# HasnainRaz/Fast-SRGAN

Hardware: AMD Instinct MI355X
Metric: SR train-step images/sec (96->384 4x, full GAN step: G+D+VGG perceptual loss) (higher is better)
Workload: dtype x3v; 1 GPU; BASELINE configs[2]: full GAN training step, 8 residual blocks / 64 filters, 96x96->384x384; per_gpu_batch=32, global_batch=32, parallelism=dp1, collectives=none, rccl_world_size=1, launch=hipGraph replay

## Files before the change

### fast-srgan_amd/_lib.py

```python
import ctypes
import os

_HERE = os.path.dirname(os.path.abspath(__file__))
LIB_PATH = os.environ.get("FSR_HIP_LIB") or os.path.join(_HERE, "libfsr_hip.so")

FSR_F32, FSR_BF16, FSR_F16, FSR_X3 = 0, 1, 2, 3
ACT_NONE, ACT_RELU, ACT_LEAKY, ACT_PRELU, ACT_TANH = 0, 1, 2, 3, 4
CONV_FWD, CONV_DGRAD = 0, 1
PACK_FWD, PACK_FWD_PS, PACK_DGRAD, PACK_DGRAD_PS = 0, 1, 2, 3
OUT_DTYPE, OUT_F32, OUT_U8, OUT_I420 = 0, 1, 2, 3
YUV_BT601, YUV_BT709 = 0, 1
SITING_JPEG, SITING_MPEG2 = 0, 1
OPT_BIAS, OPT_PRELU, OPT_OSCALE, OPT_MASK, OPT_PREACT, OPT_STATS = 1, 2, 4, 8, 16, 32
ABI_VERSION = 11

c_int, c_float, c_void_p, c_size_t, c_ll = ctypes.c_int, ctypes.c_float, ctypes.c_void_p, ctypes.c_size_t, ctypes.c_longlong


class ConvDesc(ctypes.Structure):
    _fields_ = [
        ("dtype", c_int), ("mode", c_int),
        ("n", c_int), ("ih", c_int), ("iw", c_int), ("cin", c_int),
        ("oh", c_int), ("ow", c_int), ("cout", c_int),
        ("stride", c_int), ("act", c_int), ("slope", c_float),
        ("pixel_shuffle", c_int), ("in_pixel_shuffled", c_int), ("out_f32", c_int), ("pool2", c_int), ("mask_is_addend", c_int), ("pack_lin", c_int),
        ("yuv_matrix", c_int), ("yuv_full_range", c_int),
    ]


# ... 9 lines not shown
P = c_void_p
SIGNATURES = {
    "fsr_version": (c_int, []),
    "fsr_last_error": (ctypes.c_char_p, []),
    "fsr_last_kernel": (ctypes.c_char_p, []),
    "fsr_device_info": (c_int, [ctypes.c_char_p, c_size_t]),
    "fsr_pack_conv3x3": (c_int, [c_int, c_int, P, c_int, c_int, c_int, P, P]),
    "fsr_pack_conv3x3_lin": (c_int, [c_int, c_int, P, c_int, c_int, c_int, P, P]),
    "fsr_conv3x3_pack_block": (c_int, [ctypes.POINTER(ConvDesc), c_int]),
    "fsr_conv3x3_scratch": (c_size_t, [ctypes.POINTER(ConvDesc)]),
    "fsr_conv3x3": (c_int, [ctypes.POINTER(ConvDesc), P, P, P, P, P, P, c_float, P, P, P, P, P]),
    "fsr_conv3x3_wgrad_workspace": (c_size_t, [ctypes.POINTER(WgradDesc)]),
    "fsr_conv3x3_wgrad": (c_int, [ctypes.POINTER(WgradDesc), P, P, P, P, P]),
    "fsr_conv3x3_wgrad_grouped_workspace": (c_size_t, [ctypes.POINTER(WgradDesc), c_int]),
    "fsr_conv3x3_wgrad_grouped": (c_int, [ctypes.POINTER(WgradDesc), c_int, P, P, P, P, P]),
    "fsr_instnorm_act_fwd": (c_int, [c_int, P, P, P, c_int, c_float, P, P, c_int, c_int, c_int, P]),
    "fsr_instnorm_act_bwd_scratch": (c_size_t, [c_int, c_int, c_int]),
    "fsr_instnorm_act_bwd_reduce": (c_int, [c_int, P, P, P, c_int, c_float, P, P, P, P, c_int, c_int, c_int, P]),
    "fsr_instnorm_act_bwd_apply": (c_int, [c_int, P, P, P, P, c_int, c_float, P, P, c_int, c_int, c_int, P]),
    "fsr_act_bwd_scratch": (c_size_t, [c_int, c_int, c_int, c_int, c_int]),
    "fsr_act_bwd": (c_int, [c_int, P, P, c_int, c_float, P, P, P, P, P, c_int, c_int, c_int, c_int, c_int, P]),
    "fsr_add": (c_int, [c_int, P, P, P, c_ll, P]),
    "fsr_image_to_nhwc": (c_int, [c_int, P, c_ll, c_ll, c_ll, c_ll, c_int, c_int, c_int, c_float, c_float, c_float,
                                  c_float, c_float, c_float, P, c_int, P]),
    "fsr_u8_to_image": (c_int, [P, P, c_ll, P]),
    "fsr_i420_to_image": (c_int, [P, P, c_int, c_int, c_int, c_int, c_int, c_int, P]),
    "fsr_pack_conv3x3_c3": (c_int, [c_int, P, c_int, P, c_int, P]),
    "fsr_tanh_bwd_image": (c_int, [P, c_ll, c_ll, c_ll, c_ll, P, c_int, c_int, c_int, P, P, P, P]),
    "fsr_conv3x3_c3_fwd": (c_int, [c_int, P, c_ll, c_ll, c_ll, c_ll, c_int, c_int, c_int, c_float, c_float, c_float, c_float,
                                   c_float, c_float, P, P, c_int, c_float, P, c_int, P, P, P, P]),
# ... 72 lines not shown
```

### fast-srgan_amd/csrc/conv_c3.hip

```cpp
#include "fsr_common.h"
#include "fsr_host.h"

namespace {

struct C3Args {
  const float* img;
  long long sn, sc, sh, sw;
  int N, H, W;
  float scale[3], shift[3];
  const void* wpk;
  const float* bias;
  const float* prelu;
  int act;
  float slope;
  int cout;
  void* out;
  void* preact;
  unsigned char* signs;
  const void* dz;
  float* ws;
  int tiles_x, tiles_y, tiles_per_slab, ntiles;
};

constexpr int PW = 18;
// ... 154 lines not shown
        for (int t = 0; t < 4; ++t) {
          acc[t] = (f32x4){0.f, 0.f, 0.f, 0.f};
#pragma unroll
          for (int j = 0; j < 8; ++j) acc[t] = mfma_f32_16x16x4(wf32[t][j], xv[j], acc[t]);
        }
        if (gx < a.W && gy < a.H) {
          const size_t off = (((size_t)n * a.H + gy) * a.W + gx) * a.cout + nb * 64 + lg * 8;
#pragma unroll
          for (int p = 0; p < 2; ++p) {
            const f32x4 lo = acc[2 * p] + bv[2 * p], hi = acc[2 * p + 1] + bv[2 * p + 1];
            float v8[8] = {lo[0], lo[1], lo[2], lo[3], hi[0], hi[1], hi[2], hi[3]};
            if (prep) V16<x3_t, 4>::st((x3_t*)prep + off + p * 32, v8);
#pragma unroll
            for (int q = 0; q < 8; ++q) v8[q] = fmaxf(v8[q], 0.f) + slope * fminf(v8[q], 0.f);
            V16<x3_t, 4>::st((x3_t*)outp + off + p * 32, v8);
          }
        }
        continue;
      }
    }
    static_for<0, 4>([&](auto tc) {
      constexpr int t = decltype(tc)::value;
      if (t < ntile) {
        f32x4 acc = (f32x4){0.f, 0.f, 0.f, 0.f};
        if constexpr (sizeof(T) == 2) {
          acc = mfma16<T>(wf16[t], xf16, acc);
        } else {
#pragma unroll
          for (int j = 0; j < 8; ++j) acc = mfma_f32_16x16x4(wf32[t][j], xv[j], acc);
        }
// ... 228 lines not shown
                                  void* preact, void* signs, fsr_stream_t stream_) {
  C3Args a = {};
  const float scale3[3] = {scale0, scale1, scale2}, shift3[3] = {shift0, shift1, shift2};
  if (int rc = fill_args(a, "fsr_conv3x3_c3_fwd", dtype, img, sn, sc, sh, sw, n, h, w, scale3, shift3, cout)) return rc;
  if (!packed_w || !out) return fsr_fail(-1, "fsr_conv3x3_c3_fwd: null argument");
  if (act == FSR_ACT_PRELU && !prelu_weight) return fsr_fail(-1, "fsr_conv3x3_c3_fwd: PReLU needs its weight");
  if (act == FSR_ACT_TANH) return fsr_fail(-2, "fsr_conv3x3_c3_fwd: tanh is not a first-layer activation");
  a.wpk = packed_w;
  a.bias = bias;
  a.prelu = prelu_weight;
  a.act = act;
  a.slope = slope;
  a.out = out;
  a.preact = preact;
  if (dtype == FSR_X3 && ((((size_t)out | (size_t)preact) & 127) != 0)) return fsr_fail(-2, "fsr_conv3x3_c3_fwd: x3 tensors must be 128-byte aligned");
  if (signs && (dtype == FSR_F32 || dtype == FSR_X3 || cout % 64 != 0)) return fsr_fail(-2, "fsr_conv3x3_c3_fwd: sign bits are written by the 16-bit kernels for cout %% 64 == 0");
  a.signs = (unsigned char*)signs;
  a.tiles_x = (w + 15) / 16;
  a.tiles_y = (h + 15) / 16;
  const long long nwg = (long long)a.tiles_x * a.tiles_y * n;
  if (nwg > 0x7fffffffLL) return fsr_fail(-2, "fsr_conv3x3_c3_fwd: bad grid");
  const dim3 grid((unsigned)nwg, (unsigned)((cout + 63) / 64));
  if (dtype == FSR_BF16) hipLaunchKernelGGL(conv_c3_fwd_kernel<bf16_t>, grid, dim3(256), 0, (hipStream_t)stream_, a);
  else if (dtype == FSR_F16) hipLaunchKernelGGL(conv_c3_fwd_kernel<f16_t>, grid, dim3(256), 0, (hipStream_t)stream_, a);
  else if (dtype == FSR_X3) hipLaunchKernelGGL((conv_c3_fwd_kernel<float, x3_t>), grid, dim3(256), 0, (hipStream_t)stream_, a);
  else hipLaunchKernelGGL(conv_c3_fwd_kernel<float>, grid, dim3(256), 0, (hipStream_t)stream_, a);
  return fsr_check_launch("conv_c3_fwd_kernel");
}

static int c3_wgrad_slabs(int n, int h, int w, int* tiles_x, int* tiles_y, int* per) {
  *tiles_x = (w + 15) / 16;
// ... 38 lines not shown
```

### fast-srgan_amd/csrc/conv_s2d3.hip

```cpp
#include "fsr_common.h"
#include "fsr_conv_args.h"
#include "fsr_host.h"

#include <stdlib.h>

#ifndef FSR_ABLS
#define FSR_ABLS 0
#endif

namespace {

constexpr int S2D_ABL = FSR_ABLS;

typedef float f32x16 __attribute__((ext_vector_type(16)));

template <typename T> struct Mfma32;
template <> struct Mfma32<bf16_t> {
  static __device__ __forceinline__ f32x16 run(s16x8 a, s16x8 b, f32x16 c) {
    return __builtin_amdgcn_mfma_f32_32x32x16_bf16(__builtin_bit_cast(bf16x8_hw, a), __builtin_bit_cast(bf16x8_hw, b), c, 0, 0, 0);
  }
};
template <> struct Mfma32<f16_t> {
  static __device__ __forceinline__ f32x16 run(s16x8 a, s16x8 b, f32x16 c) {
    return __builtin_amdgcn_mfma_f32_32x32x16_f16(__builtin_bit_cast(f16x8_hw, a), __builtin_bit_cast(f16x8_hw, b), c, 0, 0, 0);
// ... 381 lines not shown
    attr_set = true;
  }
  long long grid = (long long)s2d_cus() * 2;
  if (grid > a.t3_ntiles) grid = a.t3_ntiles;
  hipLaunchKernelGGL(kern, dim3((unsigned)grid), dim3(S2D_NW * 64), S2D_LDS, stream, a);
  fsr_note_kernel("conv_s2d3_kernel<%s>", X3 ? "x3" : (std::is_same<T, f16_t>::value ? "f16" : "bf16"));
  const int rc = fsr_check_launch("conv_s2d3_kernel");
  return rc ? rc : 1;
}

}

int fsr_conv_s2d3_try(int dtype, ConvKArgs& a, hipStream_t stream) {
  static const bool off = getenv("FSR_S2D3") && atoi(getenv("FSR_S2D3")) == 0;
  if (off || (dtype != FSR_BF16 && dtype != FSR_F16 && dtype != FSR_X3)) return 0;
  if (dtype == FSR_X3 && ((a.Cin & 63) != 0 || (a.Cin >> 6) * 3 >= (1 << 15) || a.dmask_bits)) return 0;
  if (a.Cin < 64 || a.Cin % 32 != 0 || a.Cout % 64 != 0 || a.Cout < 64 || a.CoutPad != a.Cout) return 0;
  if (a.ps || a.in_ps || a.out_f32 || a.preact || a.oscale || a.bias || a.stats || a.pool2 || a.act != FSR_ACT_NONE || a.dmask_add) return 0;
  if (a.IH != (a.FOH - 1) / 2 + 1 || a.IW != (a.FOW - 1) / 2 + 1) return 0;
  if ((long long)a.N * a.IH * a.IW * a.Cin >= (1LL << 31) || (long long)a.N * a.FOH * a.FOW * a.Cout >= (1LL << 31)) return 0;
  ConvKArgs b = a;
  b.tiles_x = (b.IW + 15) / 16;
  b.tiles_y = (b.IH + S2D_TH - 1) / S2D_TH;
  b.nblk_n = b.Cout / S2D_BN;
  const long long ntiles = (long long)b.tiles_x * b.tiles_y * b.N * b.nblk_n;
  if (ntiles <= 0 || ntiles > 0x7fffffffLL) return 0;
  b.t3_ntiles = (int)ntiles;
  const int want = b.Cin >= 128 ? S2D_BN : 0;
  if (b.query) {
    a.wlin_want = want;
    return 1;
// ... 9 lines not shown
```

### fast-srgan_amd/csrc/conv_tall3_body.h

```cpp
#pragma once
#include "fsr_common.h"
#include "fsr_conv_args.h"
#include "fsr_host.h"

#include <stdlib.h>

#ifndef FSR_ABL3
#define FSR_ABL3 0
#endif


int fsr_t3_cus();

namespace {

constexpr int T3_ABL = FSR_ABL3;

typedef float f32x16 __attribute__((ext_vector_type(16)));

template <typename T> struct Mfma32;
template <> struct Mfma32<bf16_t> {
  static __device__ __forceinline__ f32x16 run(s16x8 a, s16x8 b, f32x16 c) {
    return __builtin_amdgcn_mfma_f32_32x32x16_bf16(__builtin_bit_cast(bf16x8_hw, a), __builtin_bit_cast(bf16x8_hw, b), c, 0, 0, 0);
  }
// ... 402 lines not shown
        if constexpr (ACT == FSR_ACT_RELU) return fmaxf(x, 0.f);
        else if constexpr (ACT == FSR_ACT_LEAKY) return fmaxf(x, x * slope);
        else if constexpr (ACT == FSR_ACT_PRELU) return x > 0.f ? x : x * slope;
        else return x;
      };
      static_for<0, NA>([&](auto nc) {
        constexpr int n = decltype(nc)::value;
        const int co = onb * BN + wco * (NA * 32) + n * 32 + hi * 16;
        static_for<0, MB>([&](auto mc) {
          constexpr int m = decltype(mc)::value;
          const int gy = ogy0 + wpx * 2 * MB + 2 * m + lrow;
          const bool ok = gy < a.GH && gx < a.GW;
          float v[16];
#pragma unroll
          for (int e = 0; e < 16; ++e) v[e] = acc[n][m][e];
          if (a.pool2) {
#pragma unroll
            for (int e = 0; e < 16; ++e) {
              float x = v[e];
              x = fmaxf(x, __shfl_xor(x, 16, 64));
              x = fmaxf(x, __shfl_xor(x, 1, 64));
              v[e] = activate(x);
            }
            if (!(T3_ABL & 1) && ok && lrow == 0 && !(l15 & 1)) {
              const unsigned off = (unsigned)((oimg * (a.FOH >> 1) + (gy >> 1)) * (a.FOW >> 1) + (gx >> 1)) * (unsigned)a.Cout + (unsigned)co;
              store16(outp + off, v, [](float x) { return x; });
            }
          } else if (!(T3_ABL & 1) && ok) {
            unsigned off = (unsigned)((oimg * a.FOH + gy) * a.FOW + gx) * (unsigned)a.Cout + (unsigned)co;
            if constexpr (UP) {
              if (ps_out) {
                const int q = co >> a.t3_ps_shift, cc = co - (q << a.t3_ps_shift);
                off = (unsigned)((oimg * 2 * a.FOH + 2 * gy + (q >> 1)) * (2 * a.FOW) + 2 * gx + (q & 1)) * (unsigned)(a.Cout >> 2) + (unsigned)cc;
              }
              if (prep) store16(prep + off, v, [](float x) { return x; });
            }

            if (maskp) {
              const char* mp = X3 ? (const char*)x3_hi_ptr(maskp + off) : (const char*)(maskp + off);
              const u32x4 k0 = *(const u32x4*)mp, k1 = *(const u32x4*)(mp + 16);
              const float ms = a.dmask_slope;
              if (a.dmask_add) {
                if constexpr (X3) {
                  const u32x4 q0 = *(const u32x4*)(mp + 64), q1 = *(const u32x4*)(mp + 80);
#pragma unroll
                  for (int e = 0; e < 4; ++e) {
                    v[2 * e] += x3_join_lo(k0[e], q0[e]);
                    v[2 * e + 1] += x3_join_hi(k0[e], q0[e]);
                    v[8 + 2 * e] += x3_join_lo(k1[e], q1[e]);
                    v[8 + 2 * e + 1] += x3_join_hi(k1[e], q1[e]);
                  }
                } else {
#pragma unroll
// ... 134 lines not shown
```

### fast-srgan_amd/csrc/conv_wgrad.hip

```cpp
#include "fsr_common.h"
#include "fsr_host.h"
#include <cstdlib>

constexpr int WGRAD_GROUP_MAX = 32;

#ifndef FSR_ABLW
#define FSR_ABLW 0
#endif

struct WgradKArgs {
  const void* x;
  const void* dy;
  float* ws;
  int N, IH, IW, CinPad;
  int OH, OW, CoutPad;
  int dy_ps;
  int tiles_x, tiles_y, tiles_total, tiles_per_slab, nslab;
  int nbm, nbn;
  int x3;
  int group_n;
  const void* gx[WGRAD_GROUP_MAX];
  const void* gdy[WGRAD_GROUP_MAX];
};

// ... 29 lines not shown
  constexpr int PA = BM + PAD, PB = BN + PAD;
  constexpr int HH = (TPH - 1) * S + 3, HW = 15 * S + 3;
  constexpr int NPAIR = (BM / 16) * (BN / 16);
  constexpr int TPW = (NPAIR + NW - 1) / NW;
  constexpr int NBT = BN / 16;
  static_assert(TPW <= NBT, "a wave's pairs must share its co tile");
  constexpr int TPIX = TPH * 16;

  HIP_DYNAMIC_SHARED(char, smem)
  T* dyt = (T*)smem;
  T* halo = dyt + TPIX * PA;
  constexpr bool DMA = wgrad_dma<T, BM, BN, S, TPH>();

  const int tid = threadIdx.x, lane = tid & 63, wave = __builtin_amdgcn_readfirstlane(tid >> 6);
  const int l15 = lane & 15, lg = lane >> 4;
  int bid = a.group_n > 0 ? (int)blockIdx.x : xcd_remap((int)blockIdx.x, (int)gridDim.x);
  const int layer = a.group_n > 0 ? bid / a.nslab : 0;
  if (a.group_n > 0) bid -= layer * a.nslab;
  const int bn = bid % a.nbn;
  bid /= a.nbn;
  const int bm = bid % a.nbm;
  const int slab = bid / a.nbm;

  constexpr bool COPAIR = (BM >= 64 && BN == 64);
  const bool active = wave * TPW < NPAIR;
  const int co_t = COPAIR ? (wave / NBT) * TPW : (wave * TPW) / NBT;
  constexpr bool x3blk = X3W;
  const int ci_t0 = COPAIR ? (x3blk ? (wave + 2 * (wave / NBT)) % NBT : wave % NBT) : (wave * TPW) % NBT;
  const bool skip_lo = x3blk && ci_t0 >= 2;

  f32x4 acc[9][TPW];
#pragma unroll
  for (int t = 0; t < 9; ++t)
// ... 286 lines not shown
            acc[t][1] = mfma_f32_16x16x4(av1, bv, acc[t][1]);
          } else {
#pragma unroll
            for (int j = 0; j < TPW; ++j) acc[t][j] = mfma_f32_16x16x4(av, pb[j * 16], acc[t][j]);
          }
        }
      }
    }
  }

  if (!active) return;
#pragma unroll
  for (int t = 0; t < 9; ++t)
#pragma unroll
    for (int j = 0; j < TPW; ++j) {
      const int cot = COPAIR ? co_t + j : co_t, cit = COPAIR ? ci_t0 : ci_t0 + j;
      float* o = a.ws + (((size_t)(layer * a.nslab + slab) * 9 + t) * a.CoutPad + bm * BM + cot * 16 + lg * 4) * a.CinPad + bn * BN + cit * 16 + l15;
#pragma unroll
      for (int r = 0; r < 4; ++r) o[(size_t)r * a.CinPad] = acc[t][j][r];
    }
}

__global__ __launch_bounds__(256) void conv_wgrad_reduce_kernel(const float* __restrict__ ws, float* __restrict__ dw, int nslab,
                                                                int cout, int cin, int cout_pad, int cin_pad, int ps) {
  __shared__ float red[8][32];
  const int total = 9 * cout * cin;
  const size_t sstride = (size_t)9 * cout_pad * cin_pad;
  const int oi = threadIdx.x & 31, pl = threadIdx.x >> 5;
  for (int i0 = blockIdx.x * 32; i0 < total; i0 += gridDim.x * 32) {
    const int i = i0 + oi;
// ... 209 lines not shown
      const float* p = wl + ((size_t)t * cout_pad + co) * cin_pad + ci;
      for (int k = pl; k < nslab; k += 8) s += p[(size_t)k * sstride];
    }
    red[pl][oi] = s;
    __syncthreads();
    if (pl == 0 && i < total) {
      float r = red[0][oi];
#pragma unroll
      for (int j = 1; j < 8; ++j) r += red[j][oi];
      dw[((size_t)co * cin + ci) * 9 + t] += r;
    }
    __syncthreads();
  }
}

static int group_slabs(const WgradPlan& p, int nlayers) {
  int wpl = 256 / nlayers;
  if (wpl < 1) wpl = 1;
  if (wpl > p.tiles_total) wpl = p.tiles_total;
  return wpl;
}

extern "C" size_t fsr_conv3x3_wgrad_grouped_workspace(const fsr_wgrad_desc* d, int nlayers) {
  WgradPlan p;
  if (nlayers < 1 || nlayers > WGRAD_GROUP_MAX || make_plan(d, p) != 0) return 0;
  return (size_t)nlayers * group_slabs(p, nlayers) * 9 * d->cout_pad * d->cin_pad * sizeof(float);
}

extern "C" int fsr_conv3x3_wgrad_grouped(const fsr_wgrad_desc* d, int nlayers, const void* const* x, const void* const* dy,
                                         float* const* dw_oihw, void* workspace, fsr_stream_t stream_) {
  hipStream_t stream = (hipStream_t)stream_;
  WgradPlan p;
  if (int rc = make_plan(d, p)) return rc;
  if (nlayers < 1 || nlayers > WGRAD_GROUP_MAX) return fsr_fail(-2, "fsr_conv3x3_wgrad_grouped: 1..%d layers per launch", WGRAD_GROUP_MAX);
  if (!x || !dy || !dw_oihw || !workspace) return fsr_fail(-1, "fsr_conv3x3_wgrad_grouped: null argument");
// ... 72 lines not shown
  const int total = 9 * d->cout * d->cin;
  int blocks = (total + 31) / 32;
  if (blocks > 8192) blocks = 8192;
  if (x3) {
    const int total3 = 9 * d_in->cout * d_in->cin;
    int blocks3 = (total3 + 31) / 32;
    if (blocks3 > 8192) blocks3 = 8192;
    hipLaunchKernelGGL(conv_wgrad_reduce_x3_kernel, dim3(blocks3), dim3(256), 0, stream, (const float*)workspace, dw_oihw,
                       p.nslab, d_in->cout, d_in->cin, d->cout_pad, d->cin_pad, d->dy_pixel_shuffled);
    return fsr_check_launch("conv_wgrad_reduce_x3_kernel");
  }
  hipLaunchKernelGGL(conv_wgrad_reduce_kernel, dim3(blocks), dim3(256), 0, stream, (const float*)workspace, dw_oihw,
                     p.nslab, d->cout, d->cin, d->cout_pad, d->cin_pad, d->dy_pixel_shuffled);
  return fsr_check_launch("conv_wgrad_reduce_kernel");
}
```

### fast-srgan_amd/csrc/fsr_api.hip

```cpp
#include <string.h>

#include "fsr_common.h"
#include "fsr_conv_args.h"
#include "fsr_host.h"

static thread_local char g_err[512] = "";

int fsr_fail(int code, const char* fmt, ...) {
  va_list ap;
  va_start(ap, fmt);
  vsnprintf(g_err, sizeof(g_err), fmt, ap);
  va_end(ap);
  return code;
}

int fsr_check_launch(const char* what) {
  hipError_t e = hipGetLastError();
  if (e != hipSuccess) return fsr_fail(-3, "%s: launch failed: %s", what, hipGetErrorString(e));
  return 0;
}

static thread_local char g_kernel[160] = "";

void fsr_note_kernel(const char* fmt, ...) {
// ... 69 lines not shown
  ConvKArgs a;
  memset(&a, 0, sizeof(a));
  a.in = in;
  a.wpk = packed_w;
  a.out = out;
  a.bias = bias;
  a.prelu = prelu_weight;
  a.preact = preact;
  a.oscale = oscale;
  a.dmask = dact_mask;
  a.dmask_slope = dact_slope;
  a.dmask_add = (dact_mask && d->mask_is_addend == 1) ? 1 : 0;
  a.dmask_bits = (dact_mask && d->mask_is_addend == 2) ? 1 : 0;
  if (d->mask_is_addend && !dact_mask) return fsr_fail(-1, "fsr_conv3x3: mask_is_addend needs the dact_mask tensor");
  if (d->mask_is_addend < 0 || d->mask_is_addend > 2) return fsr_fail(-2, "fsr_conv3x3: mask_is_addend must be 0, 1 or 2");
  if (a.dmask_bits && (d->mode != FSR_CONV_DGRAD || d->stride != 2 || d->dtype == FSR_F32 || d->dtype == FSR_X3 || d->cout % 64 != 0))
    return fsr_fail(-2, "fsr_conv3x3: a sign-bit mask (mask_is_addend = 2) is read by the stride-2 data gradients of the 16-bit modes, cout %% 64 == 0");
  a.stats = stats ? (float*)scratch : nullptr;
  a.stats_P_max = stats ? (int)stats_slots_bound(d) : 0;
  a.query = query_block ? 1 : 0;
  a.wlin = d->pack_lin;
  if (d->pack_lin != 0 && d->pack_lin != 64 && d->pack_lin != 128) return fsr_fail(-2, "fsr_conv3x3: pack_lin must be 0, 64 or 128");
  a.N = d->n;
  a.IH = d->ih;
  a.IW = d->iw;
  a.Cin = d->dtype == FSR_X3 ? 2 * d->cin : d->cin;
  a.Cout = d->cout;
  if (d->dtype == FSR_X3) {
    if (d->cin % 32 != 0) return fsr_fail(-2, "fsr_conv3x3: x3 tensors have a multiple of 32 channels (cin = %d)", d->cin);
    if (!d->out_f32 && d->cout % 32 != 0) return fsr_fail(-2, "fsr_conv3x3: x3 tensors have a multiple of 32 channels (cout = %d)", d->cout);
    if (d->pixel_shuffle && (d->cout / 4) % 32 != 0) return fsr_fail(-2, "fsr_conv3x3: x3 pixel shuffle needs cout / 4 %% 32 == 0");
    if (d->in_pixel_shuffled && (d->cin / 4) % 32 != 0) return fsr_fail(-2, "fsr_conv3x3: x3 in_pixel_shuffled needs cin / 4 %% 32 == 0");
    if (!query_block && ((((size_t)in | (d->out_f32 ? 0 : (size_t)out) | (size_t)preact | (size_t)dact_mask) & 127) != 0))
      return fsr_fail(-2, "fsr_conv3x3: x3 tensors must be 128-byte aligned");
  }
  a.CoutPad = (d->cout + 15) / 16 * 16;
  a.FOH = d->oh;
  a.FOW = d->ow;
  a.act = d->act;
  a.slope = d->slope;
  a.ps = d->pixel_shuffle;
  a.in_ps = d->in_pixel_shuffled;
  a.out_f32 = d->out_f32;
  a.pool2 = d->pool2;
  if (d->pool2 && (d->mode != FSR_CONV_FWD || d->dtype == FSR_F32 || d->stride != 1 || d->pixel_shuffle || d->out_f32 || stats || preact ||
                   dact_mask || oscale || (d->oh & 1) || (d->ow & 1) || d->cout % 16 != 0 || d->act == FSR_ACT_TANH))
    return fsr_fail(-2, "fsr_conv3x3: pool2 is for stride-1 forward launches of the 16-bit modes with even output extents "
                        "(no statistics / pre-activation / mask / scale tensors, no pixel shuffle)");
// ... 113 lines not shown
```

### fast-srgan_amd/ops.py

```python
import ctypes
import os
import weakref

import torch

from . import _lib as L

_DT = {"f32": (L.FSR_F32, torch.float32, 16), "bf16": (L.FSR_BF16, torch.bfloat16, 32), "f16": (L.FSR_F16, torch.float16, 32),
       "x3": (L.FSR_X3, torch.float32, 32)}


class Compute:

    def __init__(self, name="f16"):
        if name not in _DT:
            raise ValueError("compute dtype must be 'bf16', 'f16', 'x3' or 'f32', got %r" % (name,))
        self.name = name
        self.code, self.torch_dtype, self.cpad = _DT[name]
        self.x3 = name == "x3"
        self.pack_dtype = torch.bfloat16 if self.x3 else self.torch_dtype
        self.pack_kmul = 2 if self.x3 else 1
        self.is16 = name in ("bf16", "f16")

    def pad(self, c):
# ... 249 lines not shown
            if _capture_seen.get(key):
                _ws_retired.append(buf)
            old = buf.numel() * 4
            nbytes = max(nbytes, 2 * old if old < (64 << 20) else old + old // 4)
        buf = torch.empty((max(nbytes, 1 << 20) + 3) // 4, dtype=torch.float32, device=device)
        _ws[key] = buf
        _capture_seen[key] = False
    if device.type == "cuda" and torch.cuda.is_current_stream_capturing():
        _capture_seen[key] = True
    return buf


_wgrad_state = {"stream": None, "active": False, "refs": [], "group": False, "pending": {}}
USE_WGRAD_STREAM = os.environ.get("FSR_WGRAD_STREAM", "1") != "0"
USE_WGRAD_GROUP = os.environ.get("FSR_WGRAD_GROUP", "1") != "0"
WGRAD_GROUP_MAX = 32


def wgrad_stream_begin(device):
    _wgrad_state["group"] = USE_WGRAD_GROUP
    if not USE_WGRAD_STREAM or L.is_emulation() or not torch.cuda.is_available():
        return
    if _wgrad_state["stream"] is None:
        _wgrad_state["stream"] = torch.cuda.Stream(device=device)
    _wgrad_state["active"] = True


def _wgrad_defer(cd, xin, dz, cout, cin, cfg, arena):
    st = _wgrad_state
    if not st["group"] or cfg.stride != 1 or cfg.pixel_shuffle or cd.x3:
        return False
    if not (cout == cin == 64 and xin.shape[3] == 64 and dz.shape[3] == 64):
        return False
    st["pending"].setdefault((cd.code, tuple(xin.shape), str(xin.device)), []).append((cd, xin, dz, arena))
    return True


def _wgrad_flush():
    st = _wgrad_state
    pending, st["pending"] = st["pending"], {}
    lib = L.lib()
    for (_code, shape, _dev), items in pending.items():
        for i0 in range(0, len(items), WGRAD_GROUP_MAX):
            grp = items[i0:i0 + WGRAD_GROUP_MAX]
            cd, x0, dz0, _ = grp[0]
            if len(grp) == 1:
                with _on_wgrad_stream(x0, dz0):
                    conv3x3_wgrad_raw(cd, x0, dz0, 64, 64, 1, out=grp[0][3])
                continue
            n, ih, iw, _c = shape
            d = L.WgradDesc(cd.code, n, ih, iw, 64, 64, ih, iw, 64, 64, 1, 0)
            need = lib.fsr_conv3x3_wgrad_grouped_workspace(ctypes.byref(d), len(grp))
            if need == 0:
                L.check(-2, "fsr_conv3x3_wgrad_grouped_workspace")
            arr = ctypes.c_void_p * len(grp)
            xs, dys, dws = arr(*[_p(g[1]) for g in grp]), arr(*[_p(g[2]) for g in grp]), arr(*[_p(g[3]) for g in grp])
            with _on_wgrad_stream(*[t for g in grp for t in (g[1], g[2])]):
                prof = PROFILE_CONV
                if prof is not None:
                    ev0, ev1 = torch.cuda.Event(enable_timing=True), torch.cuda.Event(enable_timing=True)
                    ev0.record()
                L.check(lib.fsr_conv3x3_wgrad_grouped(ctypes.byref(d), len(grp), xs, dys, dws, _p(_workspace(need, x0.device)),
                                                      _stream()), "fsr_conv3x3_wgrad_grouped")
                if prof is not None:
                    ev1.record()
                    nbytes = len(grp) * (2 * x0.numel() * x0.element_size() + 64 * 64 * 9 * 4)
                    prof.append((ev0, ev1, len(grp) * 2.0 * n * ih * iw * 64 * 64 * 9, nbytes, "conv_wgrad_kernel", "wgrad"))


def wgrad_stream_join():
    st = _wgrad_state
    if st["pending"]:
        _wgrad_flush()
    if st["active"] and st["refs"]:
        torch.cuda.current_stream().wait_stream(st["stream"])
    st["refs"] = []


# ... 142 lines not shown
        self.n_alias = n_alias
        self.emit_signs = emit_signs


class Conv3x3Fn(torch.autograd.Function):

    @staticmethod
    def forward(ctx, x, weight, bias, prelu, cfg, grad_on=True):
        ctx.grad_on = grad_on
        cd = cfg.cd
        cout, cin = weight.shape[0], weight.shape[1]
        if (cfg.image_in and cfg.stride == 1 and cout % 16 == 0 and not (cfg.pixel_shuffle or cfg.stats or cfg.tanh_head)
                and USE_C3_KERNELS):
            return Conv3x3Fn._forward_c3(ctx, x, weight, bias, prelu, cfg)
        ctx.c3 = False
        ctx.in_signs = getattr(x, "_fsr_signs", None) if (cfg.input_act_bwd is not None and cfg.stride == 2 and cd.is16) else None
        if cfg.image_in:
            xin = image_to_nhwc(cd, x, cfg.in_scale, cfg.in_shift)
        else:
            xin = x if x.is_contiguous() else x.contiguous()
            if xin.dtype != cd.torch_dtype:
                raise L.FsrError("activation dtype %s does not match the module's compute dtype %s" % (xin.dtype, cd.name))
        cin_pad = xin.shape[3]
        wpk = FilterSpec(weight, L.PACK_FWD_PS if cfg.pixel_shuffle else L.PACK_FWD, cin_pad)
        training = ctx.grad_on and any(ctx.needs_input_grad)
        if (cfg.u8_head or cfg.i420_head or cfg.pool_after) and training:
            raise L.FsrError("the uint8 / I420 head and fused max-pool epilogues are inference-only: they have no gradient")
        act = L.ACT_TANH if cfg.tanh_head else cfg.act
        want_pre = training and act == L.ACT_PRELU
        b32 = bias if bias is None or bias.dtype == torch.float32 else bias.float()
        out, pre, stats = conv3x3_raw(cd, xin, wpk, cout, stride=cfg.stride, bias=b32, act=act, slope=cfg.slope,
# ... 25 lines not shown
        cd = cfg.cd
        _check_dev(x)
        if x.dtype != torch.float32:
            x = x.float()
        n, c, h, w = x.shape
        if c != 3:
            raise ValueError("expected a 3-channel image batch, got %s" % (tuple(x.shape),))
        cout = weight.shape[0]
        wpk = packed_filter(cd, weight, PACK_C3, 32)
        training = ctx.grad_on and any(ctx.needs_input_grad)
        want_pre = training and cfg.act == L.ACT_PRELU
        b32 = bias if bias is None or bias.dtype == torch.float32 else bias.float()
        out = _empty((n, h, w, cout), cd.torch_dtype, x.device)
        pre = _empty_like(out) if want_pre else None
        signs = (torch.empty((n, h, w, cout // 8), dtype=torch.uint8, device=x.device)
                 if (cfg.emit_signs and USE_SIGN_BITS and training and cd.is16 and cout % 64 == 0) else None)
        sn, sc, sh, sw = x.stride()
        prof = PROFILE_CONV
        if prof is not None:
            ev0, ev1 = torch.cuda.Event(enable_timing=True), torch.cuda.Event(enable_timing=True)
            ev0.record()
        L.check(L.lib().fsr_conv3x3_c3_fwd(cd.code, _p(x), sn, sc, sh, sw, n, h, w, *cfg.in_scale, *cfg.in_shift, _p(wpk),
                                           _p(b32), cfg.act, float(cfg.slope), _p(prelu), cout, _p(out), _p(pre), _p(signs), _stream()),
                "fsr_conv3x3_c3_fwd")
        if signs is not None:
            out._fsr_signs = signs
        if prof is not None:
            ev1.record()
            nbytes = x.numel() * 4 + out.numel() * out.element_size() * (2 if want_pre else 1) + wpk.numel() * wpk.element_size()
            prof.append((ev0, ev1, 2.0 * n * h * w * cout * 27, nbytes, "conv_c3_fwd_kernel", "fwd"))
        ctx.cfg = cfg
# ... 412 lines not shown
```

### include/fsr_hip.h

```cpp
#ifndef FSR_HIP_H
#define FSR_HIP_H

#include <stddef.h>
#include <stdint.h>

#ifdef __cplusplus
extern "C" {
#endif

#define FSR_ABI_VERSION 11

enum { FSR_F32 = 0, FSR_BF16 = 1, FSR_F16 = 2, FSR_X3 = 3 };
enum { FSR_ACT_NONE = 0, FSR_ACT_RELU = 1, FSR_ACT_LEAKY = 2, FSR_ACT_PRELU = 3, FSR_ACT_TANH = 4 };
enum { FSR_CONV_FWD = 0, FSR_CONV_DGRAD = 1 };
enum { FSR_PACK_FWD = 0, FSR_PACK_FWD_PS = 1, FSR_PACK_DGRAD = 2, FSR_PACK_DGRAD_PS = 3 };
enum { FSR_OUT_DTYPE = 0, FSR_OUT_F32 = 1, FSR_OUT_U8 = 2, FSR_OUT_I420 = 3 };
enum { FSR_YUV_BT601 = 0, FSR_YUV_BT709 = 1 };
enum { FSR_SITING_JPEG = 0, FSR_SITING_MPEG2 = 1 };

typedef void* fsr_stream_t;

int fsr_version(void);
const char* fsr_last_error(void);
const char* fsr_last_kernel(void);
int fsr_device_info(char* buf, size_t buflen);
// ... 30 lines not shown
                void* preact, float* stats, void* scratch, fsr_stream_t stream);

typedef struct fsr_wgrad_desc {
  int dtype;
  int n, ih, iw, cin_pad, cin;
  int oh, ow, cout_pad, cout;
  int stride;
  int dy_pixel_shuffled;
} fsr_wgrad_desc;
size_t fsr_conv3x3_wgrad_workspace(const fsr_wgrad_desc* desc);
int fsr_conv3x3_wgrad(const fsr_wgrad_desc* desc, const void* x, const void* dy, float* dw_oihw, void* workspace,
                      fsr_stream_t stream);
size_t fsr_conv3x3_wgrad_grouped_workspace(const fsr_wgrad_desc* desc, int nlayers);
int fsr_conv3x3_wgrad_grouped(const fsr_wgrad_desc* desc, int nlayers, const void* const* x, const void* const* dy,
                              float* const* dw_oihw, void* workspace, fsr_stream_t stream);

int fsr_instnorm_act_fwd(int dtype, const void* x, const float* stats, const void* res, int act, float slope,
                         const float* prelu_weight, void* out, int n, int hw, int c, fsr_stream_t stream);
size_t fsr_instnorm_act_bwd_scratch(int n, int hw, int c);
int fsr_instnorm_act_bwd_reduce(int dtype, const void* g, const void* x, const float* stats, int act, float slope,
                                const float* prelu_weight, float* sums, float* dprelu, void* scratch, int n, int hw,
                                int c, fsr_stream_t stream);
int fsr_instnorm_act_bwd_apply(int dtype, const void* g, const void* x, const float* stats, const float* sums,
                               int act, float slope, const float* prelu_weight, void* dx, int n, int hw, int c,
                               fsr_stream_t stream);

size_t fsr_act_bwd_scratch(int n, int h, int w, int c, int pixel_shuffled);
int fsr_act_bwd(int dtype, const void* g, const void* saved, int act, float slope, const float* prelu_weight,
                void* dz, float* dbias, float* dprelu, void* scratch, int n, int h, int w, int c, int pixel_shuffled,
                fsr_stream_t stream);
// ... 76 lines not shown
```

Baseline: 606.7 images/s.

## Extend sign-bit masks and grouped weight-gradient batching to the x3 dtype

The c3 first-layer forward now writes packed leaky-ReLU sign bits for x3 outputs, and the stride-2 data-gradient path accepts those bit masks for x3, so the backward can read one bit per element instead of the full pre-activation mask. A new grouped x3 weight-gradient entry point batches the 64x64 stride-1 layers into one launch, with its own slab-count heuristic and a reduce kernel that sums the split hi/lo partials. The grouped x3 path is behind an environment flag that defaults off, so by default only the sign-bit change runs. The risk is correctness of the x3 sign extraction and of the hi/lo partial reduction.

```diff
diff --git a/fast-srgan_amd/_lib.py b/fast-srgan_amd/_lib.py
--- a/fast-srgan_amd/_lib.py
+++ b/fast-srgan_amd/_lib.py
@@ -12,7 +12,7 @@
 YUV_BT601, YUV_BT709 = 0, 1
 SITING_JPEG, SITING_MPEG2 = 0, 1
 OPT_BIAS, OPT_PRELU, OPT_OSCALE, OPT_MASK, OPT_PREACT, OPT_STATS = 1, 2, 4, 8, 16, 32
-ABI_VERSION = 11
+ABI_VERSION = 12
 
 c_int, c_float, c_void_p, c_size_t, c_ll = ctypes.c_int, ctypes.c_float, ctypes.c_void_p, ctypes.c_size_t, ctypes.c_longlong
 
@@ -52,6 +52,8 @@
     "fsr_conv3x3_wgrad": (c_int, [ctypes.POINTER(WgradDesc), P, P, P, P, P]),
     "fsr_conv3x3_wgrad_grouped_workspace": (c_size_t, [ctypes.POINTER(WgradDesc), c_int]),
     "fsr_conv3x3_wgrad_grouped": (c_int, [ctypes.POINTER(WgradDesc), c_int, P, P, P, P, P]),
+    "fsr_conv3x3_wgrad_grouped_x3_workspace": (c_size_t, [ctypes.POINTER(WgradDesc), c_int]),
+    "fsr_conv3x3_wgrad_grouped_x3": (c_int, [ctypes.POINTER(WgradDesc), c_int, P, P, P, P, P]),
     "fsr_instnorm_act_fwd": (c_int, [c_int, P, P, P, c_int, c_float, P, P, c_int, c_int, c_int, P]),
     "fsr_instnorm_act_bwd_scratch": (c_size_t, [c_int, c_int, c_int]),
     "fsr_instnorm_act_bwd_reduce": (c_int, [c_int, P, P, P, c_int, c_float, P, P, P, P, c_int, c_int, c_int, P]),
diff --git a/fast-srgan_amd/csrc/conv_c3.hip b/fast-srgan_amd/csrc/conv_c3.hip
--- a/fast-srgan_amd/csrc/conv_c3.hip
+++ b/fast-srgan_amd/csrc/conv_c3.hip
@@ -192,6 +192,16 @@
 #pragma unroll
             for (int q = 0; q < 8; ++q) v8[q] = fmaxf(v8[q], 0.f) + slope * fminf(v8[q], 0.f);
             V16<x3_t, 4>::st((x3_t*)outp + off + p * 32, v8);
+            if (a.signs) {
+              unsigned b = 0u;
+#pragma unroll
+              for (int q = 0; q < 4; ++q) {
+                unsigned hh, ll;
+                x3_split2(v8[2 * q], v8[2 * q + 1], hh, ll);
+                b |= ((int)(hh << 16) > 0 ? 1u << (2 * q) : 0u) | ((int)(hh & 0xffff0000u) > 0 ? 2u << (2 * q) : 0u);
+              }
+              a.signs[(((size_t)n * a.H + gy) * a.W + gx) * (a.cout >> 3) + nb * 8 + p * 4 + lg] = (unsigned char)b;
+            }
           }
         }
         continue;
@@ -450,7 +460,7 @@
   a.out = out;
   a.preact = preact;
   if (dtype == FSR_X3 && ((((size_t)out | (size_t)preact) & 127) != 0)) return fsr_fail(-2, "fsr_conv3x3_c3_fwd: x3 tensors must be 128-byte aligned");
-  if (signs && (dtype == FSR_F32 || dtype == FSR_X3 || cout % 64 != 0)) return fsr_fail(-2, "fsr_conv3x3_c3_fwd: sign bits are written by the 16-bit kernels for cout %% 64 == 0");
+  if (signs && (dtype == FSR_F32 || cout % 64 != 0)) return fsr_fail(-2, "fsr_conv3x3_c3_fwd: sign bits are written by the 16-bit and x3 kernels for cout %% 64 == 0");
   a.signs = (unsigned char*)signs;
   a.tiles_x = (w + 15) / 16;
   a.tiles_y = (h + 15) / 16;
diff --git a/fast-srgan_amd/csrc/conv_s2d3.hip b/fast-srgan_amd/csrc/conv_s2d3.hip
--- a/fast-srgan_amd/csrc/conv_s2d3.hip
+++ b/fast-srgan_amd/csrc/conv_s2d3.hip
@@ -419,7 +419,7 @@
 int fsr_conv_s2d3_try(int dtype, ConvKArgs& a, hipStream_t stream) {
   static const bool off = getenv("FSR_S2D3") && atoi(getenv("FSR_S2D3")) == 0;
   if (off || (dtype != FSR_BF16 && dtype != FSR_F16 && dtype != FSR_X3)) return 0;
-  if (dtype == FSR_X3 && ((a.Cin & 63) != 0 || (a.Cin >> 6) * 3 >= (1 << 15) || a.dmask_bits)) return 0;
+  if (dtype == FSR_X3 && ((a.Cin & 63) != 0 || (a.Cin >> 6) * 3 >= (1 << 15))) return 0;
   if (a.Cin < 64 || a.Cin % 32 != 0 || a.Cout % 64 != 0 || a.Cout < 64 || a.CoutPad != a.Cout) return 0;
   if (a.ps || a.in_ps || a.out_f32 || a.preact || a.oscale || a.bias || a.stats || a.pool2 || a.act != FSR_ACT_NONE || a.dmask_add) return 0;
   if (a.IH != (a.FOH - 1) / 2 + 1 || a.IW != (a.FOW - 1) / 2 + 1) return 0;
diff --git a/fast-srgan_amd/csrc/conv_tall3_body.h b/fast-srgan_amd/csrc/conv_tall3_body.h
--- a/fast-srgan_amd/csrc/conv_tall3_body.h
+++ b/fast-srgan_amd/csrc/conv_tall3_body.h
@@ -440,7 +440,7 @@
           float v[16];
 #pragma unroll
           for (int e = 0; e < 16; ++e) v[e] = acc[n][m][e];
-          if (a.pool2) {
+          if (!UP && a.pool2) {
 #pragma unroll
             for (int e = 0; e < 16; ++e) {
               float x = v[e];
@@ -462,7 +462,7 @@
               if (prep) store16(prep + off, v, [](float x) { return x; });
             }
 
-            if (maskp) {
+            if (!UP && maskp) {
               const char* mp = X3 ? (const char*)x3_hi_ptr(maskp + off) : (const char*)(maskp + off);
               const u32x4 k0 = *(const u32x4*)mp, k1 = *(const u32x4*)(mp + 16);
               const float ms = a.dmask_slope;
diff --git a/fast-srgan_amd/csrc/conv_wgrad.hip b/fast-srgan_amd/csrc/conv_wgrad.hip
--- a/fast-srgan_amd/csrc/conv_wgrad.hip
+++ b/fast-srgan_amd/csrc/conv_wgrad.hip
@@ -67,9 +67,10 @@
 
   const int tid = threadIdx.x, lane = tid & 63, wave = __builtin_amdgcn_readfirstlane(tid >> 6);
   const int l15 = lane & 15, lg = lane >> 4;
-  int bid = a.group_n > 0 ? (int)blockIdx.x : xcd_remap((int)blockIdx.x, (int)gridDim.x);
-  const int layer = a.group_n > 0 ? bid / a.nslab : 0;
-  if (a.group_n > 0) bid -= layer * a.nslab;
+  int bid = (a.group_n > 0 && a.nbm * a.nbn == 1) ? (int)blockIdx.x : xcd_remap((int)blockIdx.x, (int)gridDim.x);
+  const int per_layer = a.nslab * a.nbm * a.nbn;
+  const int layer = a.group_n > 0 ? bid / per_layer : 0;
+  if (a.group_n > 0) bid -= layer * per_layer;
   const int bn = bid % a.nbn;
   bid /= a.nbn;
   const int bm = bid % a.nbm;
@@ -386,6 +387,7 @@
   for (int t = 0; t < 9; ++t)
 #pragma unroll
     for (int j = 0; j < TPW; ++j) {
+      if (X3W && j >= 2 && skip_lo) continue;
       const int cot = COPAIR ? co_t + j : co_t, cit = COPAIR ? ci_t0 : ci_t0 + j;
       float* o = a.ws + (((size_t)(layer * a.nslab + slab) * 9 + t) * a.CoutPad + bm * BM + cot * 16 + lg * 4) * a.CinPad + bn * BN + cit * 16 + l15;
 #pragma unroll
@@ -625,11 +627,76 @@
   }
 }
 
+__global__ __launch_bounds__(256) void conv_wgrad_reduce_x3_grouped_kernel(const float* __restrict__ ws, const WgradGroupOut out, int nslab,
+                                                                           int cout, int cin, int cout_pad, int cin_pad) {
+  __shared__ float red[8][32];
+  const int total = 9 * cout * cin;
+  const size_t sstride = (size_t)9 * cout_pad * cin_pad;
+  const int oi = threadIdx.x & 31, pl = threadIdx.x >> 5;
+  const float* wl = ws + (size_t)blockIdx.y * nslab * sstride;
+  float* dw = out.dw[0];
+#pragma unroll
+  for (int l = 1; l < WGRAD_GROUP_MAX; ++l)
+    if (l == (int)blockIdx.y) dw = out.dw[l];
+  for (int i0 = blockIdx.x * 32; i0 < total; i0 += gridDim.x * 32) {
+    const int i = i0 + oi;
+    float s = 0.f;
+    int co = 0, ci = 0, t = 0;
+    if (i < total) {
+      ci = i % cin;
+      co = (i / cin) % cout;
+      t = i / (cin * cout);
+      const int rh = (co >> 5) * 64 + (co & 31), ch = (ci >> 5) * 64 + (ci & 31);
+      const float* p = wl + ((size_t)t * cout_pad + rh) * cin_pad + ch;
+      const size_t rlo = (size_t)32 * cin_pad;
+      float hh = 0.f, hl = 0.f, lh = 0.f;
+      for (int k = pl; k < nslab; k += 8) {
+        const float* q = p + (size_t)k * sstride;
+        hh += q[0];
+        hl += q[32];
+        lh += q[rlo];
+      }
+      s = hh + (hl + lh);
+    }
+    red[pl][oi] = s;
+    __syncthreads();
+    if (pl == 0 && i < total) {
+      float r = red[0][oi];
+#pragma unroll
+      for (int j = 1; j < 8; ++j) r += red[j][oi];
+      dw[((size_t)co * cin + ci) * 9 + t] += r;
+    }
+    __syncthreads();
+  }
+}
+
 static int group_slabs(const WgradPlan& p, int nlayers) {
   int wpl = 256 / nlayers;
   if (wpl < 1) wpl = 1;
   if (wpl > p.tiles_total) wpl = p.tiles_total;
   return wpl;
+}
+
+static int group_slabs_x3(const WgradPlan& p, int nlayers) {
+  const int per_slab = nlayers * p.nbm * p.nbn;
+  int best = 1;
+  long best_cost = -1;
+  for (int r = 1; r <= 4; ++r) {
+    int ns = r * 256 / per_slab;
+    if (ns < 1) ns = 1;
+    if (ns > p.tiles_total) ns = p.tiles_total;
+    const int rounds = (ns * per_slab + 255) / 256;
+    const long cost = (long)rounds * ((p.tiles_total + ns - 1) / ns);
+    if (best_cost < 0 || cost < best_cost) {
+      best_cost = cost;
+      best = ns;
+    }
+  }
+  if (const char* e = getenv("FSR_WGRAD_SLABS")) {
+    const int v = atoi(e);
+    if (v > 0) best = v < p.tiles_total ? v : p.tiles_total;
+  }
+  return best;
 }
 
 extern "C" size_t fsr_conv3x3_wgrad_grouped_workspace(const fsr_wgrad_desc* d, int nlayers) {
@@ -732,3 +799,49 @@
                      p.nslab, d->cout, d->cin, d->cout_pad, d->cin_pad, d->dy_pixel_shuffled);
   return fsr_check_launch("conv_wgrad_reduce_kernel");
 }
+
+extern "C" size_t fsr_conv3x3_wgrad_grouped_x3_workspace(const fsr_wgrad_desc* d, int nlayers) {
+  WgradPlan p;
+  if (nlayers < 1 || nlayers > WGRAD_GROUP_MAX || !d || d->dtype != FSR_X3 || make_plan(d, p) != 0) return 0;
+  return (size_t)nlayers * group_slabs_x3(p, nlayers) * 9 * d->cout_pad * d->cin_pad * 4 * sizeof(float);
+}
+
+extern "C" int fsr_conv3x3_wgrad_grouped_x3(const fsr_wgrad_desc* d_in, int nlayers, const void* const* x, const void* const* dy,
+                                            float* const* dw_oihw, void* workspace, fsr_stream_t stream_) {
+  hipStream_t stream = (hipStream_t)stream_;
+  WgradPlan p;
+  if (int rc = make_plan(d_in, p)) return rc;
+  if (d_in->dtype != FSR_X3) return fsr_fail(-2, "fsr_conv3x3_wgrad_grouped_x3: x3 tensors only (fsr_conv3x3_wgrad_grouped serves the other types)");
+  if (nlayers < 1 || nlayers > WGRAD_GROUP_MAX) return fsr_fail(-2, "fsr_conv3x3_wgrad_grouped_x3: 1..%d layers per launch", WGRAD_GROUP_MAX);
+  if (!x || !dy || !dw_oihw || !workspace) return fsr_fail(-1, "fsr_conv3x3_wgrad_grouped_x3: null argument");
+  if (d_in->stride != 1 || d_in->dy_pixel_shuffled || d_in->cout != 64 || d_in->cin != 64 || d_in->cout_pad != 64 || d_in->cin_pad != 64)
+    return fsr_fail(-2, "fsr_conv3x3_wgrad_grouped_x3: layers with cout = cin = 64, unpadded, stride 1, no pixel shuffle");
+  const fsr_wgrad_desc dphys = physical_desc(d_in);
+  const fsr_wgrad_desc* d = &dphys;
+  WgradKArgs a = {};
+  WgradGroupOut out = {};
+  for (int l = 0; l < nlayers; ++l) {
+    if (!x[l] || !dy[l] || !dw_oihw[l]) return fsr_fail(-1, "fsr_conv3x3_wgrad_grouped_x3: null pointer for layer %d", l);
+    if ((((size_t)x[l] | (size_t)dy[l]) & 127) != 0) return fsr_fail(-2, "fsr_conv3x3_wgrad_grouped_x3: x3 tensors must be 128-byte aligned");
+    a.gx[l] = x[l];
+    a.gdy[l] = dy[l];
+    out.dw[l] = dw_oihw[l];
+  }
+  a.group_n = nlayers;
+  a.x3 = 1;
+  a.ws = (float*)workspace;
+  a.N = d->n; a.IH = d->ih; a.IW = d->iw; a.CinPad = d->cin_pad;
+  a.OH = d->oh; a.OW = d->ow; a.CoutPad = d->cout_pad;
+  a.dy_ps = 0;
+  a.tiles_x = p.tiles_x; a.tiles_y = p.tiles_y; a.tiles_total = p.tiles_total;
+  a.nslab = group_slabs_x3(p, nlayers);
+  a.tiles_per_slab = (p.tiles_total + a.nslab - 1) / a.nslab;
+  a.nslab = (p.tiles_total + a.tiles_per_slab - 1) / a.tiles_per_slab;
+  a.nbm = p.nbm;
+  a.nbn = p.nbn;
+  if (int rc = dispatch_wgrad<bf16_t, 8>(p, a, stream)) return rc;
+  const int total = 9 * d_in->cout * d_in->cin;
+  hipLaunchKernelGGL(conv_wgrad_reduce_x3_grouped_kernel, dim3((total + 31) / 32, nlayers), dim3(256), 0, stream, (const float*)workspace, out,
+                     a.nslab, d_in->cout, d_in->cin, d->cout_pad, d->cin_pad);
+  return fsr_check_launch("conv_wgrad_reduce_x3_grouped_kernel");
+}
diff --git a/fast-srgan_amd/csrc/fsr_api.hip b/fast-srgan_amd/csrc/fsr_api.hip
--- a/fast-srgan_amd/csrc/fsr_api.hip
+++ b/fast-srgan_amd/csrc/fsr_api.hip
@@ -107,8 +107,8 @@
   a.dmask_bits = (dact_mask && d->mask_is_addend == 2) ? 1 : 0;
   if (d->mask_is_addend && !dact_mask) return fsr_fail(-1, "fsr_conv3x3: mask_is_addend needs the dact_mask tensor");
   if (d->mask_is_addend < 0 || d->mask_is_addend > 2) return fsr_fail(-2, "fsr_conv3x3: mask_is_addend must be 0, 1 or 2");
-  if (a.dmask_bits && (d->mode != FSR_CONV_DGRAD || d->stride != 2 || d->dtype == FSR_F32 || d->dtype == FSR_X3 || d->cout % 64 != 0))
-    return fsr_fail(-2, "fsr_conv3x3: a sign-bit mask (mask_is_addend = 2) is read by the stride-2 data gradients of the 16-bit modes, cout %% 64 == 0");
+  if (a.dmask_bits && (d->mode != FSR_CONV_DGRAD || d->stride != 2 || d->dtype == FSR_F32 || d->cout % 64 != 0))
+    return fsr_fail(-2, "fsr_conv3x3: a sign-bit mask (mask_is_addend = 2) is read by the stride-2 data gradients of the 16-bit and x3 modes, cout %% 64 == 0");
   a.stats = stats ? (float*)scratch : nullptr;
   a.stats_P_max = stats ? (int)stats_slots_bound(d) : 0;
   a.query = query_block ? 1 : 0;
@@ -124,7 +124,7 @@
     if (!d->out_f32 && d->cout % 32 != 0) return fsr_fail(-2, "fsr_conv3x3: x3 tensors have a multiple of 32 channels (cout = %d)", d->cout);
     if (d->pixel_shuffle && (d->cout / 4) % 32 != 0) return fsr_fail(-2, "fsr_conv3x3: x3 pixel shuffle needs cout / 4 %% 32 == 0");
     if (d->in_pixel_shuffled && (d->cin / 4) % 32 != 0) return fsr_fail(-2, "fsr_conv3x3: x3 in_pixel_shuffled needs cin / 4 %% 32 == 0");
-    if (!query_block && ((((size_t)in | (d->out_f32 ? 0 : (size_t)out) | (size_t)preact | (size_t)dact_mask) & 127) != 0))
+    if (!query_block && ((((size_t)in | (d->out_f32 ? 0 : (size_t)out) | (size_t)preact | (a.dmask_bits ? 0 : (size_t)dact_mask)) & 127) != 0))
       return fsr_fail(-2, "fsr_conv3x3: x3 tensors must be 128-byte aligned");
   }
   a.CoutPad = (d->cout + 15) / 16 * 16;
diff --git a/fast-srgan_amd/ops.py b/fast-srgan_amd/ops.py
--- a/fast-srgan_amd/ops.py
+++ b/fast-srgan_amd/ops.py
@@ -287,6 +287,7 @@
 _wgrad_state = {"stream": None, "active": False, "refs": [], "group": False, "pending": {}}
 USE_WGRAD_STREAM = os.environ.get("FSR_WGRAD_STREAM", "1") != "0"
 USE_WGRAD_GROUP = os.environ.get("FSR_WGRAD_GROUP", "1") != "0"
+USE_WGRAD_GROUP_X3 = os.environ.get("FSR_WGRAD_GROUP_X3", "0") == "1"
 WGRAD_GROUP_MAX = 32
 
 
@@ -301,10 +302,12 @@
 
 def _wgrad_defer(cd, xin, dz, cout, cin, cfg, arena):
     st = _wgrad_state
-    if not st["group"] or cfg.stride != 1 or cfg.pixel_shuffle or cd.x3:
+    if not st["group"] or cfg.stride != 1 or cfg.pixel_shuffle or (cd.x3 and not USE_WGRAD_GROUP_X3):
         return False
     if not (cout == cin == 64 and xin.shape[3] == 64 and dz.shape[3] == 64):
         return False
+    if cd.x3:
+        xin, dz = _aligned(xin), _aligned(dz)
     st["pending"].setdefault((cd.code, tuple(xin.shape), str(xin.device)), []).append((cd, xin, dz, arena))
     return True
 
@@ -323,9 +326,12 @@
                 continue
             n, ih, iw, _c = shape
             d = L.WgradDesc(cd.code, n, ih, iw, 64, 64, ih, iw, 64, 64, 1, 0)
-            need = lib.fsr_conv3x3_wgrad_grouped_workspace(ctypes.byref(d), len(grp))
+            ws_fn, fn, what = ((lib.fsr_conv3x3_wgrad_grouped_x3_workspace, lib.fsr_conv3x3_wgrad_grouped_x3, "fsr_conv3x3_wgrad_grouped_x3")
+                               if cd.x3 else
+                               (lib.fsr_conv3x3_wgrad_grouped_workspace, lib.fsr_conv3x3_wgrad_grouped, "fsr_conv3x3_wgrad_grouped"))
+            need = ws_fn(ctypes.byref(d), len(grp))
             if need == 0:
-                L.check(-2, "fsr_conv3x3_wgrad_grouped_workspace")
+                L.check(-2, what + "_workspace")
             arr = ctypes.c_void_p * len(grp)
             xs, dys, dws = arr(*[_p(g[1]) for g in grp]), arr(*[_p(g[2]) for g in grp]), arr(*[_p(g[3]) for g in grp])
             with _on_wgrad_stream(*[t for g in grp for t in (g[1], g[2])]):
@@ -333,8 +339,7 @@
                 if prof is not None:
                     ev0, ev1 = torch.cuda.Event(enable_timing=True), torch.cuda.Event(enable_timing=True)
                     ev0.record()
-                L.check(lib.fsr_conv3x3_wgrad_grouped(ctypes.byref(d), len(grp), xs, dys, dws, _p(_workspace(need, x0.device)),
-                                                      _stream()), "fsr_conv3x3_wgrad_grouped")
+                L.check(fn(ctypes.byref(d), len(grp), xs, dys, dws, _p(_workspace(need, x0.device)), _stream()), what)
                 if prof is not None:
                     ev1.record()
                     nbytes = len(grp) * (2 * x0.numel() * x0.element_size() + 64 * 64 * 9 * 4)
@@ -507,7 +512,7 @@
                 and USE_C3_KERNELS):
             return Conv3x3Fn._forward_c3(ctx, x, weight, bias, prelu, cfg)
         ctx.c3 = False
-        ctx.in_signs = getattr(x, "_fsr_signs", None) if (cfg.input_act_bwd is not None and cfg.stride == 2 and cd.is16) else None
+        ctx.in_signs = getattr(x, "_fsr_signs", None) if (cfg.input_act_bwd is not None and cfg.stride == 2 and (cd.is16 or cd.x3)) else None
         if cfg.image_in:
             xin = image_to_nhwc(cd, x, cfg.in_scale, cfg.in_shift)
         else:
@@ -563,7 +568,7 @@
         out = _empty((n, h, w, cout), cd.torch_dtype, x.device)
         pre = _empty_like(out) if want_pre else None
         signs = (torch.empty((n, h, w, cout // 8), dtype=torch.uint8, device=x.device)
-                 if (cfg.emit_signs and USE_SIGN_BITS and training and cd.is16 and cout % 64 == 0) else None)
+                 if (cfg.emit_signs and USE_SIGN_BITS and training and (cd.is16 or cd.x3) and cout % 64 == 0) else None)
         sn, sc, sh, sw = x.stride()
         prof = PROFILE_CONV
         if prof is not None:
diff --git a/include/fsr_hip.h b/include/fsr_hip.h
--- a/include/fsr_hip.h
+++ b/include/fsr_hip.h
@@ -8,7 +8,7 @@
 extern "C" {
 #endif
 
-#define FSR_ABI_VERSION 11
+#define FSR_ABI_VERSION 12
 
 enum { FSR_F32 = 0, FSR_BF16 = 1, FSR_F16 = 2, FSR_X3 = 3 };
 enum { FSR_ACT_NONE = 0, FSR_ACT_RELU = 1, FSR_ACT_LEAKY = 2, FSR_ACT_PRELU = 3, FSR_ACT_TANH = 4 };
@@ -69,6 +69,9 @@
 size_t fsr_conv3x3_wgrad_grouped_workspace(const fsr_wgrad_desc* desc, int nlayers);
 int fsr_conv3x3_wgrad_grouped(const fsr_wgrad_desc* desc, int nlayers, const void* const* x, const void* const* dy,
                               float* const* dw_oihw, void* workspace, fsr_stream_t stream);
+size_t fsr_conv3x3_wgrad_grouped_x3_workspace(const fsr_wgrad_desc* desc, int nlayers);
+int fsr_conv3x3_wgrad_grouped_x3(const fsr_wgrad_desc* desc, int nlayers, const void* const* x, const void* const* dy,
+                                 float* const* dw_oihw, void* workspace, fsr_stream_t stream);
 
 int fsr_instnorm_act_fwd(int dtype, const void* x, const float* stats, const void* res, int act, float slope,
                          const float* prelu_weight, void* out, int n, int hw, int c, fsr_stream_t stream);
```

Measured after the change: 611.7 images/s (median of 6 runs). Within noise of the previous version (+0.8%).
